# filaPro/unidet3d

Hardware: AMD Instinct MI355X
Metric: scenes/sec fwd+bwd, 100k-pt ScanNet voxel grid, 1/2/4/8 MI355X (higher is better)
Workload: dtype f32

## Files before the change

### unidet3d_amd/csrc/bn.hip

```cpp
#include <stdlib.h>

#include "u3d_common.h"

namespace u3d {

struct BnFin {
    double* sums;
    double rows;
    int set_rows;
    const float* gamma;
    const float* beta;
    float eps, momentum;
    float* running_mean;
    float* running_var;
    float* st;
    int64_t* nbt;
};

__device__ __forceinline__ void bn_finalize_channel(double s1, double s2, double rows, const float* gamma, const float* beta, float eps,
                                                    float momentum, float* running_mean, float* running_var, float* mean, float* invstd,
                                                    float* scale, float* shift, int c) {
#pragma clang fp contract(off)
    const double m = s1 / rows;
    double var = fma(-m, m, s2 / rows);
    if (var < 0.0) var = 0.0;
    const float is = (float)(1.0 / sqrt(var + (double)eps));
    const float mf = (float)m;
    mean[c] = mf;
    invstd[c] = is;
    const float sc = gamma[c] * is;
    scale[c] = sc;
    shift[c] = fmaf(-mf, sc, beta[c]);
    if (running_mean) {
        const double unbiased = rows > 1.0 ? var * rows / (rows - 1.0) : var;
        const float keep = 1.f - momentum;
        const float km = keep * running_mean[c], kv = keep * running_var[c];
        const float nm = momentum * mf, nv = momentum * (float)unbiased;
        running_mean[c] = km + nm;
        running_var[c] = kv + nv;
    }
}

__device__ __forceinline__ void bn_finish_body(const double* partial, int nblk, int C, const BnFin& f, int wave0, int nw, bool first) {
    const int lane = threadIdx.x & 63;
    for (int c = wave0; c < C; c += nw) {
        double t1 = 0.0, t2 = 0.0;
        for (int b = lane; b < nblk; b += 64) {
            t1 += partial[(int64_t)b * 2 * C + c];
            t2 += partial[(int64_t)b * 2 * C + C + c];
        }
#pragma unroll
        for (int d = 32; d >= 1; d >>= 1) { t1 += __shfl_xor(t1, d, 64); t2 += __shfl_xor(t2, d, 64); }
        if (lane) continue;
        f.sums[c] = t1;
        f.sums[C + c] = t2;
        if (!f.st) continue;
        bn_finalize_channel(t1, t2, f.rows, f.gamma, f.beta, f.eps, f.momentum, f.running_mean, f.running_var, f.st, f.st + C,
                            f.st + 2 * C, f.st + 3 * C, c);
    }
    if (first && threadIdx.x == 0) {
        if (f.set_rows) f.sums[2 * C] = f.rows;
        if (f.nbt) *f.nbt += 1;
    }
}

__global__ __launch_bounds__(256) void bn_sum_k(const double* __restrict__ partial, int nblk, int C, BnFin f) {
    bn_finish_body(partial, nblk, C, f, blockIdx.x * 4 + (threadIdx.x >> 6), gridDim.x * 4, blockIdx.x == 0);
}

template <int MODE>
__global__ __launch_bounds__(256) void bn_reduce_k(const float* __restrict__ x, const float* __restrict__ dy,
                                                   const float* __restrict__ mean, const float* __restrict__ invstd,
                                                   const float* __restrict__ scale, const float* __restrict__ shift, int relu,
                                                   int64_t n, int C, double* sums ) {
    __shared__ double sh[256 * 8];
    const int lpr = C >> 2;
    const int rpb = 256 / lpr;
    const int tid = threadIdx.x;
    const int c4 = tid % lpr, slot = tid / lpr;
    double a[4] = {0, 0, 0, 0}, b[4] = {0, 0, 0, 0};
    if (slot < rpb) {
        float4 mu = make_float4(0, 0, 0, 0), is = mu, sc = mu, sf = mu;
        if (MODE == 1) {
            mu = *reinterpret_cast<const float4*>(mean + c4 * 4);
            is = *reinterpret_cast<const float4*>(invstd + c4 * 4);
            sc = *reinterpret_cast<const float4*>(scale + c4 * 4);
            sf = *reinterpret_cast<const float4*>(shift + c4 * 4);
        }
        const int64_t stride = (int64_t)gridDim.x * rpb;
        for (int64_t r0 = (int64_t)blockIdx.x * rpb + slot; r0 < n; r0 += 4 * stride) {
            float4 v4[4], g4[4];
#pragma unroll
            for (int u = 0; u < 4; ++u) {
                const int64_t r = r0 + u * stride;
                v4[u] = make_float4(0.f, 0.f, 0.f, 0.f);
                g4[u] = make_float4(0.f, 0.f, 0.f, 0.f);
                if (r < n) {
                    v4[u] = *reinterpret_cast<const float4*>(x + r * C + c4 * 4);
                    if (MODE == 1) g4[u] = *reinterpret_cast<const float4*>(dy + r * C + c4 * 4);
                }
            }
#pragma unroll
            for (int u = 0; u < 4; ++u) {
                const float4 v = v4[u];
                if (MODE == 0) {
                    a[0] += v.x; a[1] += v.y; a[2] += v.z; a[3] += v.w;
                    b[0] += (double)v.x * v.x; b[1] += (double)v.y * v.y; b[2] += (double)v.z * v.z; b[3] += (double)v.w * v.w;
                } else {
                    float4 g = g4[u];
                    if (relu) {
                        if (!(v.x * sc.x + sf.x > 0.f)) g.x = 0.f;
                        if (!(v.y * sc.y + sf.y > 0.f)) g.y = 0.f;
                        if (!(v.z * sc.z + sf.z > 0.f)) g.z = 0.f;
                        if (!(v.w * sc.w + sf.w > 0.f)) g.w = 0.f;
                    }
                    a[0] += g.x; a[1] += g.y; a[2] += g.z; a[3] += g.w;
                    b[0] += (double)g.x * ((v.x - mu.x) * is.x); b[1] += (double)g.y * ((v.y - mu.y) * is.y);
                    b[2] += (double)g.z * ((v.z - mu.z) * is.z); b[3] += (double)g.w * ((v.w - mu.w) * is.w);
                }
            }
        }
    }
#pragma unroll
    for (int j = 0; j < 4; ++j) { sh[tid * 8 + j] = a[j]; sh[tid * 8 + 4 + j] = b[j]; }
    __syncthreads();
    if (tid < lpr) {
        double ta[4] = {0, 0, 0, 0}, tb[4] = {0, 0, 0, 0};
        for (int s = 0; s < rpb; ++s) {
            const int o = (s * lpr + tid) * 8;
#pragma unroll
            for (int j = 0; j < 4; ++j) { ta[j] += sh[o + j]; tb[j] += sh[o + 4 + j]; }
        }
        double* out = sums + (int64_t)blockIdx.x * 2 * C;
// ... 39 lines not shown
                              float* running_var, int C, float* mean, float* invstd, float* scale, float* shift,
                              int64_t* num_batches_tracked) {
    const int c = blockIdx.x * blockDim.x + threadIdx.x;
    if (c == 0 && num_batches_tracked) *num_batches_tracked += 1;
    if (c >= C) return;
    if (!(count > 0.0)) count = sums[2 * C];
    bn_finalize_channel(sums[c], sums[C + c], count, gamma, beta, eps, momentum, running_mean, running_var, mean, invstd, scale, shift, c);
}


__global__ __launch_bounds__(256) void bn_apply_k(const float* __restrict__ x, const float* __restrict__ scale,
                                                  const float* __restrict__ shift, int relu, int64_t n4, int C4, float* y, __bf16* yb) {
    for (int64_t i = (int64_t)blockIdx.x * blockDim.x + threadIdx.x; i < n4; i += (int64_t)gridDim.x * blockDim.x) {
        const int c4 = (int)(i % C4);
        const float4 v = reinterpret_cast<const float4*>(x)[i];
        const float4 sc = reinterpret_cast<const float4*>(scale)[c4];
        const float4 sf = reinterpret_cast<const float4*>(shift)[c4];
        const float4 o = bn_affine_relu(v, sc, sf, relu);
        reinterpret_cast<float4*>(y)[i] = o;
        if (yb) store_shadow(yb, i / C4, C4, 0, c4, o);
    }
}

__global__ __launch_bounds__(256) void bn_bwd_apply_k(const float* __restrict__ x, const float* __restrict__ dy,
                                                      const float* __restrict__ mean, const float* __restrict__ invstd,
                                                      const float* __restrict__ scale, const float* __restrict__ shift, int relu,
                                                      const double* __restrict__ sums, double inv_count, int64_t n4, int C,
                                                      float* dx, float* dgamma, float* dbeta, const double* __restrict__ count_src,
                                                      const float* __restrict__ addend, __bf16* dxb) {
    const int C4 = C >> 2;
    if (!(inv_count > 0.0)) inv_count = 1.0 / (count_src ? count_src[0] : sums[2 * C]);
    if (blockIdx.x == 0 && dgamma) {
        for (int c = threadIdx.x; c < C; c += blockDim.x) {
            dbeta[c] = (float)sums[c];
            dgamma[c] = (float)sums[C + c];
        }
    }
    for (int64_t i = (int64_t)blockIdx.x * blockDim.x + threadIdx.x; i < n4; i += (int64_t)gridDim.x * blockDim.x) {
        const int c4 = (int)(i % C4);
        const float4 v = reinterpret_cast<const float4*>(x)[i];
        float4 g = reinterpret_cast<const float4*>(dy)[i];
        const float4 mu = reinterpret_cast<const float4*>(mean)[c4];
        const float4 is = reinterpret_cast<const float4*>(invstd)[c4];
        const float4 sc = reinterpret_cast<const float4*>(scale)[c4];
        const float4 sf = reinterpret_cast<const float4*>(shift)[c4];
        if (relu) {
            if (!(v.x * sc.x + sf.x > 0.f)) g.x = 0.f;
            if (!(v.y * sc.y + sf.y > 0.f)) g.y = 0.f;
            if (!(v.z * sc.z + sf.z > 0.f)) g.z = 0.f;
            if (!(v.w * sc.w + sf.w > 0.f)) g.w = 0.f;
        }
        const int c = c4 * 4;
        const float m1x = (float)(sums[c] * inv_count), m1y = (float)(sums[c + 1] * inv_count);
        const float m1z = (float)(sums[c + 2] * inv_count), m1w = (float)(sums[c + 3] * inv_count);
        const float m2x = (float)(sums[C + c] * inv_count), m2y = (float)(sums[C + c + 1] * inv_count);
        const float m2z = (float)(sums[C + c + 2] * inv_count), m2w = (float)(sums[C + c + 3] * inv_count);
        float4 o;
        o.x = sc.x * (g.x - m1x - (v.x - mu.x) * is.x * m2x);
        o.y = sc.y * (g.y - m1y - (v.y - mu.y) * is.y * m2y);
        o.z = sc.z * (g.z - m1z - (v.z - mu.z) * is.z * m2z);
        o.w = sc.w * (g.w - m1w - (v.w - mu.w) * is.w * m2w);
        if (addend) {
            const float4 e = reinterpret_cast<const float4*>(addend)[i];
            o.x += e.x; o.y += e.y; o.z += e.z; o.w += e.w;
        }
        reinterpret_cast<float4*>(dx)[i] = o;
        if (dxb) store_shadow(dxb, i / C4, C4, 0, c4, o);
    }
}

static bool bn_ok(int64_t n, int C) { return n > 0 && C >= 4 && C <= 512 && C % 4 == 0; }
static bool shadow_ok(const void* sh, int C) { return !sh || C % 32 == 0; }
static unsigned ew_grid(int64_t n4) {
    int64_t g = ceil_div(n4, 256);
    return (unsigned)(g < 1 ? 1 : (g > 4096 ? 4096 : g));
}

}

using namespace u3d;

extern "C" {

static int bn_grid(int64_t n, int C) {
    const int rpb = 256 / (C / 4);
    int64_t g = ceil_div(n, (int64_t)rpb * 16);
    return (int)(g < 1 ? 1 : (g > 256 ? 256 : g));
}
static int bn_partials_grid(int64_t n_tiles, int C) {
    const int rpp = 2 * C >= 256 ? 1 : 256 / (2 * C);
    int64_t g = ceil_div(n_tiles, (int64_t)rpp * 16);
    return (int)(g < 1 ? 1 : (g > 128 ? 128 : g));
}

int64_t u3d_bn_ws_bytes(int C) { return (int64_t)256 * 2 * C * sizeof(double) + 64; }

static int bn_finish_launch(const void* ws, int nblk, int C, const BnFin& f, hipStream_t s) {
    hipLaunchKernelGGL(bn_sum_k, dim3((C + 3) / 4), dim3(256), 0, s, (const double*)ws, nblk, C, f);
    return check_launch("bn_sum");
}

static BnFin bn_fin(double* sums, double rows, int set_rows) {
    BnFin f;
    f.sums = sums; f.rows = rows; f.set_rows = set_rows; f.gamma = nullptr; f.beta = nullptr; f.eps = 0.f; f.momentum = 0.f;
    f.running_mean = nullptr; f.running_var = nullptr; f.st = nullptr; f.nbt = nullptr;
    return f;
}

static int bn_stats_launch(const float* x, int64_t n, int C, const float* partial, int64_t n_tiles, const BnFin& f, void* ws, hipStream_t s) {
    if (partial) {
        if (n_tiles <= 0) return U3D_EINVAL;
        ProfScope prof(U3D_K_BN, s, (double)n_tiles * C * 8);
        const int g = bn_partials_grid(n_tiles, C);
        hipLaunchKernelGGL(bn_partials_k, dim3(g), dim3(256), 0, s, partial, n_tiles, C, (double*)ws);
        return bn_finish_launch(ws, g, C, f, s);
    }
    ProfScope prof(U3D_K_BN, s, (double)n * C * 4);
    const int g = bn_grid(n, C);
    hipLaunchKernelGGL(bn_reduce_k<0>, dim3(g), dim3(256), 0, s, x, (const float*)nullptr, (const float*)nullptr,
                       (const float*)nullptr, (const float*)nullptr, (const float*)nullptr, 0, n, C, (double*)ws);
    return bn_finish_launch(ws, g, C, f, s);
}

int u3d_bn_stats(const float* x, int64_t n, int C, const float* partial, int64_t n_tiles, double* sums, void* ws, u3d_stream_t stream) {
    if ((!x && !partial) || !sums || !ws || !bn_ok(n, C)) return U3D_EINVAL;
    return bn_stats_launch(x, n, C, partial, n_tiles, bn_fin(sums, (double)n, 1), ws, (hipStream_t)stream);
}

int u3d_bn_finalize(const double* sums, double count, const float* gamma, const float* beta, float eps, float momentum,
                    float* running_mean, float* running_var, int C, float* mean, float* invstd, float* scale,
                    float* shift, int64_t* num_batches_tracked, u3d_stream_t stream) {
    if (!sums || !gamma || !beta || !mean || !invstd || !scale || !shift || C <= 0) return U3D_EINVAL;
    hipLaunchKernelGGL(bn_finalize_k, dim3((C + 63) / 64), dim3(64), 0, (hipStream_t)stream, sums, count, gamma, beta, eps,
                       momentum, running_mean, running_var, C, mean, invstd, scale, shift, num_batches_tracked);
    return check_launch("bn_finalize");
}

int u3d_bn_apply(const float* x, const float* scale, const float* shift, int relu, int64_t n, int C, float* y, void* y_bf16,
                 u3d_stream_t stream) {
    if (!x || !scale || !shift || !y || !bn_ok(n, C) || !shadow_ok(y_bf16, C)) return U3D_EINVAL;
    hipStream_t s = (hipStream_t)stream;
    ProfScope prof(U3D_K_BN, s, (double)n * C * (y_bf16 ? 10 : 8));
    const int64_t n4 = n * (C / 4);
    hipLaunchKernelGGL(bn_apply_k, dim3(ew_grid(n4)), dim3(256), 0, s, x, scale, shift, relu, n4, C / 4, y, (__bf16*)y_bf16);
    return check_launch("bn_apply");
}

int u3d_bn_bwd_stats(const float* x, const float* dy, const float* mean, const float* invstd, const float* scale,
                     const float* shift, int relu, int64_t n, int C, double* sums, void* ws, u3d_stream_t stream) {
    if (!x || !dy || !mean || !invstd || !scale || !shift || !sums || !ws || !bn_ok(n, C)) return U3D_EINVAL;
    hipStream_t s = (hipStream_t)stream;
    ProfScope prof(U3D_K_BN, s, (double)n * C * 8);
    const int g = bn_grid(n, C);
    const BnFin f = bn_fin(sums, 0.0, 0);
    hipLaunchKernelGGL(bn_reduce_k<1>, dim3(g), dim3(256), 0, s, x, dy, mean, invstd, scale, shift, relu, n, C, (double*)ws);
    return bn_finish_launch(ws, g, C, f, s);
}

int u3d_bn_bwd_apply(const float* x, const float* dy, const float* mean, const float* invstd, const float* scale,
                     const float* shift, int relu, const double* sums, double count, int64_t n, int C, float* dx, void* dx_bf16,
                     float* dgamma, float* dbeta, const float* addend, u3d_stream_t stream) {
    if (!x || !dy || !mean || !invstd || !scale || !shift || !sums || !dx || !bn_ok(n, C) || !shadow_ok(dx_bf16, C)) return U3D_EINVAL;
    hipStream_t s = (hipStream_t)stream;
    ProfScope prof(U3D_K_BN, s, (double)n * C * 12);
    const int64_t n4 = n * (C / 4);
    hipLaunchKernelGGL(bn_bwd_apply_k, dim3(ew_grid(n4)), dim3(256), 0, s, x, dy, mean, invstd, scale, shift, relu, sums,
                       1.0 / count, n4, C, dx, dgamma, dbeta, (const double*)nullptr, addend, (__bf16*)dx_bf16);
    return check_launch("bn_bwd_apply");
}

int u3d_bn_forward(const float* x, int64_t n, int C, const float* partial, int64_t n_tiles, const float* gamma, const float* beta, float eps,
                   float momentum, float* running_mean, float* running_var, int64_t* num_batches_tracked, int relu, float* y, void* y_bf16,
                   float* st, double* sums, void* ws, u3d_stream_t stream) {
    if (!x || !sums || !ws || !gamma || !beta || !st || !y || !bn_ok(n, C) || !shadow_ok(y_bf16, C)) return U3D_EINVAL;
    if (partial && n_tiles <= 0) return U3D_EINVAL;
    BnFin f = bn_fin(sums, (double)n, 1);
    f.gamma = gamma; f.beta = beta; f.eps = eps; f.momentum = momentum; f.running_mean = running_mean; f.running_var = running_var;
    f.st = st; f.nbt = num_batches_tracked;
    int rc = bn_stats_launch(x, n, C, partial, n_tiles, f, ws, (hipStream_t)stream);
    if (rc) return rc;
    return u3d_bn_apply(x, st + 2 * C, st + 3 * C, relu, n, C, y, y_bf16, stream);
}

int u3d_bn_backward(const float* x, const float* dy, const float* st, int relu, const double* fwd_sums, double* sums, int64_t n, int C,
                    float* dx, void* dx_bf16, float* dgamma, float* dbeta, const float* addend, void* ws, u3d_stream_t stream) {
    if (!fwd_sums || !st || !dx || !shadow_ok(dx_bf16, C)) return U3D_EINVAL;
    int rc = u3d_bn_bwd_stats(x, dy, st, st + C, st + 2 * C, st + 3 * C, relu, n, C, sums, ws, stream);
    if (rc) return rc;
    hipStream_t s = (hipStream_t)stream;
    ProfScope prof(U3D_K_BN, s, (double)n * C * 12);
    const int64_t n4 = n * (C / 4);
    hipLaunchKernelGGL(bn_bwd_apply_k, dim3(ew_grid(n4)), dim3(256), 0, s, x, dy, (const float*)st, (const float*)(st + C), (const float*)(st + 2 * C),
                       (const float*)(st + 3 * C), relu, (const double*)sums, -1.0, n4, C, dx, dgamma, dbeta, fwd_sums + 2 * C, addend,
                       (__bf16*)dx_bf16);
    return check_launch("bn_backward");
}

}
```

### unidet3d_amd/csrc/gemm.hip

```cpp
#include "gemm_common.h"

namespace u3d {

#define U3D_MFMA32(a, b, c) __builtin_amdgcn_mfma_f32_32x32x2f32((a), (b), (c), 0, 0, 0)

constexpr int GLD = GK + 4;


template <int TN, int EPI, int TM = GT>
__global__ __launch_bounds__(256) void gemm_nt_k(const float* __restrict__ A, const float* __restrict__ W, const float* __restrict__ bias,
                                                 float* __restrict__ C, int64_t M, int N, int K, const float* __restrict__ aux,
                                                 float* __restrict__ pre) {
    constexpr int NB = TN / 64, TA = TM / 64;
    __shared__ __attribute__((aligned(16))) float As[2][TM * GLD];
    __shared__ __attribute__((aligned(16))) float Bs[2][TN * GLD];
    const int tid = threadIdx.x, lane = tid & 63;
    const int wave = __builtin_amdgcn_readfirstlane(tid >> 6);
    const int wr = wave >> 1, wc = wave & 1, i32 = lane & 31, kh = lane >> 5;
    const int nt_ = (N + TN - 1) / TN;
    const int64_t wid_ = xcd_swizzle(blockIdx.x, gridDim.x);
    const int64_t m0 = (wid_ / nt_) * TM;
    const int n0 = (int)(wid_ % nt_) * TN;
    const int rows_a = (int)min((int64_t)TM, M - m0), rows_b = min(TN, N - n0);
    const __amdgpu_buffer_rsrc_t rs_a = make_rsrc(A + m0 * K, (int64_t)rows_a * K * 4);
// ... 473 lines not shown
    auto gload = [&](int t) {
#pragma unroll
        for (int j = 0; j < 4; ++j) {
            ra[j] = bload128(rs_a, ca ? va + j * 8 * N * 4 : va, t * (TKH * N * 4));
            rb[j] = bload128(rs_b, cb ? vb + j * 8 * K * 4 : vb, t * (TKH * K * 4));
        }
    };
    auto lstore = [&](int buf) {
#pragma unroll
        for (int j = 0; j < 4; ++j) {
            cs += ra[j];
            *reinterpret_cast<bf16x4*>(&As[buf][(srow + 8 * j) * TLH + sc4 * 4]) = bf16x4{(__bf16)ra[j][0], (__bf16)ra[j][1], (__bf16)ra[j][2], (__bf16)ra[j][3]};
            *reinterpret_cast<bf16x4*>(&Bs[buf][(srow + 8 * j) * TLH + sc4 * 4]) = bf16x4{(__bf16)rb[j][0], (__bf16)rb[j][1], (__bf16)rb[j][2], (__bf16)rb[j][3]};
        }
    };
    const int troff = ((lane & 15) >> 2) * TLH + 16 * ((lane >> 4) & 1) + 4 * (lane & 3);
    auto colfrag = [&](const __bf16* t, int row0, int col32) {
        const __bf16* p = t + row0 * TLH + col32 + troff;
        return tr16_pair(p, p + 4 * TLH);
    };
    f32x16 acc[2][2];
#pragma unroll
    for (int a = 0; a < 2; ++a)
#pragma unroll
        for (int b = 0; b < 2; ++b)
#pragma unroll
            for (int r = 0; r < 16; ++r) acc[a][b][r] = 0.f;
    const int nt = (rows + TKH - 1) / TKH;
    if (nt > 0) {
        gload(0);
        lstore(0);
    }
    __syncthreads();
    for (int t = 0; t < nt; ++t) {
        const int buf = t & 1;
        if (t + 1 < nt) gload(t + 1);
#pragma unroll
        for (int h = 0; h < 2; ++h) {
            const int r0 = h * 16 + kh * 8;
            bf16x8 af[2], bf[2];
#pragma unroll
            for (int u = 0; u < 2; ++u) {
                af[u] = colfrag(As[buf], r0, wr * 64 + u * 32);
                bf[u] = colfrag(Bs[buf], r0, wc * 64 + u * 32);
            }
#pragma unroll
            for (int a = 0; a < 2; ++a)
#pragma unroll
                for (int b = 0; b < 2; ++b) acc[a][b] = __builtin_amdgcn_mfma_f32_32x32x16_bf16(af[a], bf[b], acc[a][b], 0, 0, 0);
        }
        if (t + 1 < nt) lstore(buf ^ 1);
        __syncthreads();
    }
    const int64_t pstride = (int64_t)N * K + (colsum ? N : 0);
    const __amdgpu_buffer_rsrc_t rs_o = make_rsrc(partial + (int64_t)blockIdx.z * pstride, (int64_t)N * K * 4);
#pragma unroll
    for (int b = 0; b < 2; ++b) {
        const int k = k0 + wc * 64 + b * 32 + i32;
        const int vo = k < K ? ((n0 + 4 * kh) * K + k) * 4 : 0x7fffffff;
#pragma unroll
        for (int a = 0; a < 2; ++a)
#pragma unroll
            for (int r = 0; r < 16; ++r) {
                const int row = wr * 64 + a * 32 + (r & 3) + 8 * (r >> 2);
                float v = acc[a][b][r];
                asm volatile("" : "+v"(v));
                __builtin_amdgcn_raw_buffer_store_b32(__builtin_bit_cast(unsigned, v), rs_o, vo, row * K * 4, 0);
            }
    }
    if (colsum && blockIdx.y == 0) {
#pragma unroll
        for (int c = 0; c < 4; ++c) csum_s[srow][sc4 * 4 + c] = cs[c];
        __syncthreads();
        if (tid < GT && n0 + tid < N) {
            float v = 0.f;
#pragma unroll
            for (int r = 0; r < 8; ++r) v += csum_s[r][tid];
            partial[(int64_t)blockIdx.z * pstride + (int64_t)N * K + n0 + tid] = v;
        }
    }
}

__global__ __launch_bounds__(256) void gemm_tn_reduce_k(const float* __restrict__ partial, int S, int64_t n4, int64_t n4_main, float* __restrict__ C,
                                                        float* __restrict__ C2) {
    for (int64_t i = (int64_t)blockIdx.x * blockDim.x + threadIdx.x; i < n4; i += (int64_t)gridDim.x * blockDim.x) {
        float4 v[4];
#pragma unroll
        for (int u = 0; u < 4; ++u) v[u] = make_float4(0.f, 0.f, 0.f, 0.f);
        int s = 0;
        for (; s + 4 <= S; s += 4) {
#pragma unroll
            for (int u = 0; u < 4; ++u) {
                const float4 t = reinterpret_cast<const float4*>(partial)[(int64_t)(s + u) * n4 + i];
                v[u].x += t.x; v[u].y += t.y; v[u].z += t.z; v[u].w += t.w;
            }
        }
        for (; s < S; ++s) {
            const float4 t = reinterpret_cast<const float4*>(partial)[(int64_t)s * n4 + i];
            v[0].x += t.x; v[0].y += t.y; v[0].z += t.z; v[0].w += t.w;
        }
        float4* dst = i < n4_main ? reinterpret_cast<float4*>(C) + i : reinterpret_cast<float4*>(C2) + (i - n4_main);
        *dst = make_float4((v[0].x + v[1].x) + (v[2].x + v[3].x), (v[0].y + v[1].y) + (v[2].y + v[3].y),
                                                      (v[0].z + v[1].z) + (v[2].z + v[3].z), (v[0].w + v[1].w) + (v[2].w + v[3].w));
    }
}

void launch_tn_reduce(const float* ws, int S, int N, int K, float* C, float* colsum, hipStream_t s) {
    const int64_t n4_main = (int64_t)N * K / 4, n4 = n4_main + (colsum ? N / 4 : 0);
    int64_t grid = ceil_div(n4, 256);
    grid = grid > 1024 ? 1024 : grid;
    hipLaunchKernelGGL(gemm_tn_reduce_k, dim3((unsigned)grid), dim3(256), 0, s, ws, S, n4, n4_main, C, colsum);
}

__global__ __launch_bounds__(256) void gelu_fwd_k(const float4* __restrict__ h, float4* __restrict__ a, int64_t n4) {
    for (int64_t i = (int64_t)blockIdx.x * blockDim.x + threadIdx.x; i < n4; i += (int64_t)gridDim.x * blockDim.x) {
        const float4 v = h[i];
        a[i] = make_float4(gelu_f(v.x), gelu_f(v.y), gelu_f(v.z), gelu_f(v.w));
    }
}
__global__ __launch_bounds__(256) void gelu_bwd_k(const float4* __restrict__ da, const float4* __restrict__ h, float4* __restrict__ dh, int64_t n4) {
    for (int64_t i = (int64_t)blockIdx.x * blockDim.x + threadIdx.x; i < n4; i += (int64_t)gridDim.x * blockDim.x) {
        const float4 g = da[i], v = h[i];
        dh[i] = make_float4(g.x * gelu_grad_f(v.x), g.y * gelu_grad_f(v.y), g.z * gelu_grad_f(v.z), g.w * gelu_grad_f(v.w));
    }
}

__global__ __launch_bounds__(256) void transpose_k(const float* __restrict__ in, float* __restrict__ out, int R, int Ccols) {
    __shared__ float tile[32][33];
    const int bx = blockIdx.x * 32, by = blockIdx.y * 32;
    const int tx = threadIdx.x & 31, ty = threadIdx.x >> 5;
    for (int j = ty; j < 32; j += 8)
        if (by + j < R && bx + tx < Ccols) tile[j][tx] = in[(int64_t)(by + j) * Ccols + bx + tx];
    __syncthreads();
    for (int j = ty; j < 32; j += 8)
        if (bx + j < Ccols && by + tx < R) out[(int64_t)(bx + j) * R + by + tx] = tile[tx][j];
}

struct TrDesc { const float* src; float* dst; int64_t R, C, block0; };
__global__ __launch_bounds__(256) void transpose_batch_k(const TrDesc* __restrict__ desc, int n_desc) {
    __shared__ float tile[32][33];
    int lo = 0, hi = n_desc;
    while (hi - lo > 1) {
        const int mid = (lo + hi) >> 1;
        if (desc[mid].block0 <= (int64_t)blockIdx.x) lo = mid; else hi = mid;
    }
    const TrDesc d = desc[lo];
    const int R = (int)d.R, Ccols = (int)d.C;
    const int tiles_x = (Ccols + 31) / 32;
    const int rem = (int)((int64_t)blockIdx.x - d.block0);
    const int bx = (rem % tiles_x) * 32, by = (rem / tiles_x) * 32;
    const int tx = threadIdx.x & 31, ty = threadIdx.x >> 5;
    for (int j = ty; j < 32; j += 8)
        if (by + j < R && bx + tx < Ccols) tile[j][tx] = d.src[(int64_t)(by + j) * Ccols + bx + tx];
    __syncthreads();
    for (int j = ty; j < 32; j += 8)
        if (bx + j < Ccols && by + tx < R) d.dst[(int64_t)(bx + j) * R + by + tx] = tile[tx][j];
}

struct PlDesc { const float* src; bf16x8* dst; int64_t n8, block0; };
__global__ __launch_bounds__(256) void planes_batch_k(const PlDesc* __restrict__ desc, int n_desc) {
    int lo = 0, hi = n_desc;
    while (hi - lo > 1) {
        const int mid = (lo + hi) >> 1;
        if (desc[mid].block0 <= (int64_t)blockIdx.x) lo = mid; else hi = mid;
    }
    const PlDesc d = desc[lo];
    const int64_t idx = ((int64_t)blockIdx.x - d.block0) * 256 + threadIdx.x;
    if (idx >= d.n8) return;
    const f32x4 a = *reinterpret_cast<const f32x4*>(d.src + idx * 8), b = *reinterpret_cast<const f32x4*>(d.src + idx * 8 + 4);
    bf16x8 out[3];
    split3_x8(a, b, out);
#pragma unroll
    for (int q = 0; q < 3; ++q) d.dst[q * d.n8 + idx] = out[q];
}

static int tn_tile(int N, int K) { return ceil_div(N, GT) * ceil_div(K, GT) < 16 ? 64 : GT; }
static int tn_splits(int64_t M, int N, int K, int T, bool bf) {
    const int64_t tiles = ceil_div(N, T) * ceil_div(K, T);
    static const int target = [] { const char* e = getenv("U3D_TN_WGS"); return e && atoi(e) > 0 ? atoi(e) : 768; }();
    return tn_clamp_splits(ceil_div(bf ? 384 : target, tiles), M, GK);
}

static int nt_plan(int64_t M, int N, int K, bool bf, NtPlan* plan) {
    if (M <= 0 || N <= 0 || K <= 0) return U3D_EINVAL;
    const bool x3 = !bf && fp32_x3() && K % GKH == 0;
    if (K % (bf ? GKH : GK)) { set_error("gemm_nt: K=%d must be a multiple of %d", K, bf ? GKH : GK); return U3D_EUNSUPPORTED; }
    if (!nt_offsets_ok("gemm_nt", N, K)) return U3D_EUNSUPPORTED;
    static const int force = [] { const char* e = getenv("U3D_NT_TILE"); return e ? atoi(e) : 0; }();
    const double over[3] = {1.0, 1.04, 1.08};
    int best = 0;
    double best_t = 0.0;
    for (int c = x3 ? 1 : 0; c < 3; ++c) {
        const int64_t wgs = ceil_div(M, NT_TM[c]) * ceil_div(N, NT_TN[c]);
        const double t = (double)ceil_div(wgs, 256) * NT_TM[c] * NT_TN[c] * over[c];
// ... 220 lines not shown
```

### unidet3d_amd/csrc/spconv.hip

```cpp
#include <stdlib.h>

#include "u3d_common.h"
#include "spconv_gmm.h"

namespace u3d {

#ifndef U3D_GMM_ABL
#define U3D_GMM_ABL 0
#endif
#ifndef U3D_WG_ABL
#define U3D_WG_ABL 0
#endif
__device__ __forceinline__ int gmm_acc_idx(int r, int c4) { return GMM_SWZ ? r * 32 + ((c4 ^ (r & 7)) << 2) : r * GMM_ALD + (c4 << 2); }

template <int NI, int JB, int NW = 2>
struct GmmBuf {
    f32x4 a[NI];
    f32x4 b[JB][NW];
};

struct GmmItem {
    int k, base, e;
    bool valid;
};
// ... 626 lines not shown
                    for (int b = 0; b < NXW; ++b) asm volatile("" :: "v"(xv[u][b]));
                }
                return;
            }
#pragma unroll
            for (int u = 0; u < 4; ++u)
#pragma unroll
                for (int a = 0; a < NGW; ++a)
#pragma unroll
                    for (int b = 0; b < NXW; ++b) acc[a][b] = __builtin_amdgcn_mfma_f32_16x16x4f32(gv[u][a], xv[u][b], acc[a][b], 0, 0, 0);
        };
        load_idx(ioA, ixA, base);
        load_idx(ioB, ixB, min(base + 16, last));
        load_rows(gA, xA, ioA, ixA);
        for (int t = 0; t < nfull; t += 2) {
            load_rows(gB, xB, ioB, ixB);
            load_idx(ioA, ixA, min(base + (t + 2) * 16, last));
            mfmas(gA, xA);
            if (t + 1 >= nfull) break;
            load_rows(gA, xA, ioA, ixA);
            load_idx(ioB, ixB, min(base + (t + 3) * 16, last));
            mfmas(gB, xB);
        }
        base += nfull * 16;
    }
    if (base < hi) {
        float gv[4][NGW], xv[4][NXW];
#pragma unroll
        for (int u = 0; u < 4; ++u) {
            const int pi = min(base + 4 * q + u, hi - 1);
            const int io = bload32(rs_rg, pi * 4, ksoff), ix = bload32(rs_rx, pi * 4, ksoff);
            load_row_part<NGW>(gv[u], rs_g, (int)__umul24(io, CD * 4) + gvo);
            load_row_part<NXW>(xv[u], rs_x, (int)__umul24(ix, CS * 4) + xvo);
        }
#pragma unroll
        for (int u = 0; u < 4; ++u) {
            const bool ok = base + 4 * q + u < hi;
#pragma unroll
            for (int a = 0; a < NGW; ++a) {
                const float ga = ok ? gv[u][a] : 0.f;
#pragma unroll
                for (int b = 0; b < NXW; ++b) acc[a][b] = __builtin_amdgcn_mfma_f32_16x16x4f32(ga, xv[u][b], acc[a][b], 0, 0, 0);
            }
        }
    }
    if constexpr (LDSR) {
        constexpr int EW = NGW * NXW * 256;
        __shared__ float red[2][EW];
        float* mine = red[wave & 1] + lane;
        if (wave < 2) {
#pragma unroll
            for (int a = 0; a < NGW; ++a)
#pragma unroll
                for (int b = 0; b < NXW; ++b)
#pragma unroll
                    for (int r = 0; r < 4; ++r) mine[((a * NXW + b) * 4 + r) * 64] = acc[a][b][r];
        }
        __syncthreads();
        if (wave >= 2) {
#pragma unroll
            for (int a = 0; a < NGW; ++a)
#pragma unroll
                for (int b = 0; b < NXW; ++b)
#pragma unroll
                    for (int r = 0; r < 4; ++r) mine[((a * NXW + b) * 4 + r) * 64] += acc[a][b][r];
        }
        __syncthreads();
        const int group = range >> 2;
        if ((range & ~3) >= p.n_tiles) return;
        float* out = p.partial + ((int64_t)k * ceil_div(p.n_tiles, 4) + group) * (CD * CS);
        for (int e = threadIdx.x; e < EW; e += 256) out[e] = red[0][e] + red[1][e];
        return;
    }
    float* out = p.partial + ((int64_t)k * p.n_tiles + range) * (CD * CS) + (int64_t)sub * (NGW * NXW * 256) + lane;
#pragma unroll
    for (int a = 0; a < NGW; ++a)
#pragma unroll
        for (int b = 0; b < NXW; ++b)
#pragma unroll
            for (int r = 0; r < 4; ++r) out[((a * NXW + b) * 4 + r) * 64] = acc[a][b][r];
}

__global__ __launch_bounds__(256) void wgrad_reduce_k(const float* __restrict__ partial, int n_tiles, int K, int NG, int NX, int SG, int SX,
                                                      float* __restrict__ dW) {
    const int CS = NX * 16, E = NG * NX * 256;
    const int k = blockIdx.y;
    const int idx = blockIdx.x * 256 + threadIdx.x;
    if (idx >= E) return;
    const float* src = partial + (int64_t)k * n_tiles * E + idx;
    float v0 = 0.f, v1 = 0.f, v2 = 0.f, v3 = 0.f;
    int r = 0;
    for (; r + 4 <= n_tiles; r += 4) {
        v0 += src[(int64_t)r * E];
        v1 += src[(int64_t)(r + 1) * E];
        v2 += src[(int64_t)(r + 2) * E];
        v3 += src[(int64_t)(r + 3) * E];
    }
    for (; r < n_tiles; ++r) v0 += src[(int64_t)r * E];
    const float v = (v0 + v1) + (v2 + v3);
    const int NGW = NG / SG, NXW = NX / SX, per_sub = NGW * NXW * 256;
    const int sub = idx / per_sub, rem = idx % per_sub;
    const int e = rem >> 6, lane = rem & 63, i16 = lane & 15, q = lane >> 4;
    const int rr = e & 3, b = (e >> 2) % NXW, a = (e >> 2) / NXW;
    const int wa = sub % SG, wb = sub / SG;
    const int co = NG * (4 * q + rr) + wa * NGW + a, ci = NX * i16 + wb * NXW + b;
    dW[((int64_t)co * K + k) * CS + ci] = v;
}

static int plan_wgrad_rows(int K, int64_t n_rows, int Cs, int Cd) {
    static const int64_t cap = [] { const char* e = getenv("U3D_WGRAD_TILES"); const int64_t v = e ? atoll(e) : 0; return v > 0 ? v : (int64_t)256; }();
    static const int64_t budget = [] { const char* e = getenv("U3D_WGRAD_PARTIAL_MB"); const int64_t v = e ? atoll(e) : 0; return (v > 0 ? v : (int64_t)64) << 20; }();
    int64_t nt = budget / ((int64_t)K * Cs * Cd * 4);
    const int64_t rows_per = (K >= 27 && Cs == 32 && Cd == 32) ? 520 : 1300;
    const int64_t cap_n = cap > n_rows / rows_per ? cap : n_rows / rows_per;
    nt = nt > cap_n ? cap_n : (nt < 1 ? 1 : nt);
    const int64_t by_len = ceil_div(n_rows, 64);
    if (nt > by_len) nt = by_len;
    return (int)ceil_div(n_rows, nt);
}

template <int NX, int NG, int PR = 0>
static int launch_wgrad(const WgParams& p0, float* dW, hipStream_t s) {
    constexpr int SG = (NG * NX > 32 && NG % 2 == 0 && NG >= NX) ? 2 : ((NG * NX > 64 && NG % 2 == 0) ? 2 : 1);
    constexpr int SX = ((NG / SG) * NX > 32 && NX % 2 == 0) ? 2 : 1;
    constexpr int SPLIT = SG * SX, RPW = 4 / SPLIT;
    static_assert(SPLIT == 1 || SPLIT == 2 || SPLIT == 4, "wave split");
    const WgParams& p = p0;
    const int64_t groups = ceil_div(ceil_div(p.n_tiles, RPW), 8) * 8;
    static const int pipe_env = [] { const char* e = getenv("U3D_WGRAD_PIPE"); return e ? atoi(e) : -1; }();
    const bool pipe = pipe_env >= 0 ? pipe_env != 0 : (NG / SG) * (NX / SX) <= 16;
    if (pipe) hipLaunchKernelGGL((spconv_wgrad_k<NG, NX, SG, SX, PR, true>), dim3((unsigned)(groups * p.K)), dim3(256), 0, s, p);
    else hipLaunchKernelGGL((spconv_wgrad_k<NG, NX, SG, SX, PR, false>), dim3((unsigned)(groups * p.K)), dim3(256), 0, s, p);
    const int n_blocks = SPLIT == 1 ? (int)ceil_div(p.n_tiles, 4) : p.n_tiles;
    hipLaunchKernelGGL(wgrad_reduce_k, dim3(NG * NX, p.K), dim3(256), 0, s, (const float*)p.partial, n_blocks, p.K, NG, NX, SG, SX, dW);
    return check_launch("spconv_wgrad");
}

static inline int64_t weight_pack_vectors(int format, int Cd, int K, int Cs) { return (int64_t)(Cd / 32) * K * (Cs / (format ? 32 : 16)) * 2 * 64; }

__device__ __forceinline__ void weight_f32_vector(const float* __restrict__ w, float* __restrict__ wp, int64_t idx, int Cd, int K, int Cs, int transposed) {
    const int lane = (int)(idx & 63);
    int64_t t = idx >> 6;
    const int nb = (int)(t & 1); t >>= 1;
    const int cs16 = Cs / 16;
    if (idx >= (int64_t)(Cd / 32) * K * cs16 * 2 * 64) return;
    const int j = (int)(t % cs16); t /= cs16;
    const int k = (int)(t % K);
    const int slice = (int)(t / K);
    const int n = slice * 32 + nb * 16 + (lane & 15), c = j * 16 + (lane >> 4) * 4;
    float4 v;
    if (!transposed) {
        v = *reinterpret_cast<const float4*>(w + ((int64_t)n * K + k) * Cs + c);
    } else {
        v.x = w[((int64_t)(c + 0) * K + k) * Cd + n];
        v.y = w[((int64_t)(c + 1) * K + k) * Cd + n];
        v.z = w[((int64_t)(c + 2) * K + k) * Cd + n];
        v.w = w[((int64_t)(c + 3) * K + k) * Cd + n];
    }
    reinterpret_cast<float4*>(wp)[idx] = v;
}

__device__ __forceinline__ void weight_bf16_vector(const float* __restrict__ w, bf16x8* __restrict__ wp, int64_t idx, int Cd, int K, int Cs, int transposed) {
    const int lane = (int)(idx & 63);
    int64_t t = idx >> 6;
    const int nb = (int)(t & 1); t >>= 1;
    const int cs32 = Cs / 32;
    if (idx >= (int64_t)(Cd / 32) * K * cs32 * 2 * 64) return;
    const int jj = (int)(t % cs32); t /= cs32;
    const int k = (int)(t % K);
    const int slice = (int)(t / K);
    const int n = slice * 32 + nb * 16 + (lane & 15), q = lane >> 4;
    bf16x8 v;
#pragma unroll
    for (int e = 0; e < 8; ++e) {
        const int c = (2 * jj + (e >> 2)) * 16 + q * 4 + (e & 3);
        v[e] = (__bf16)(transposed ? w[((int64_t)c * K + k) * Cd + n] : w[((int64_t)n * K + k) * Cs + c]);
    }
    wp[idx] = v;
}

__device__ __forceinline__ void weight_x3_vectors(const float* __restrict__ w, bf16x8* __restrict__ wp, int64_t idx, int Cd, int K, int Cs, int transposed) {
    if (idx >= (int64_t)(Cd / 32) * K * (Cs / 32) * 2 * 64) return;
    const int cs32 = Cs / 32;
    const int lane = (int)(idx & 63);
    int64_t t = idx >> 6;
    const int nb = (int)(t & 1); t >>= 1;
    const int jj = (int)(t % cs32); t /= cs32;
    const int k = (int)(t % K);
    const int slice = (int)(t / K);
    const int n = slice * 32 + nb * 16 + (lane & 15), q = lane >> 4;
    float v[8];
#pragma unroll
    for (int e = 0; e < 8; ++e) {
        const int c = (2 * jj + (e >> 2)) * 16 + q * 4 + (e & 3);
        v[e] = transposed ? w[((int64_t)c * K + k) * Cd + n] : w[((int64_t)n * K + k) * Cs + c];
    }
    bf16x8 pl[3];
    split3_x8(f32x4{v[0], v[1], v[2], v[3]}, f32x4{v[4], v[5], v[6], v[7]}, pl);
    const int64_t o = (idx >> 6) * 192 + lane;
#pragma unroll
    for (int pq = 0; pq < 3; ++pq) wp[o + pq * 64] = pl[pq];
}
__device__ __forceinline__ void weight_pack_vector(int64_t format, const float* w, void* wp, int64_t idx, int Cd, int K, int Cs, int transposed) {
    if (format == 2) weight_x3_vectors(w, reinterpret_cast<bf16x8*>(wp), idx, Cd, K, Cs, transposed);
    else if (format) weight_bf16_vector(w, reinterpret_cast<bf16x8*>(wp), idx, Cd, K, Cs, transposed);
    else weight_f32_vector(w, reinterpret_cast<float*>(wp), idx, Cd, K, Cs, transposed);
}

template <int FORMAT>
__global__ __launch_bounds__(256) void weight_pack_k(const float* __restrict__ w, void* __restrict__ wp, int Cd, int K, int Cs, int transposed) {
    weight_pack_vector(FORMAT, w, wp, (int64_t)blockIdx.x * blockDim.x + threadIdx.x, Cd, K, Cs, transposed);
}

struct PackDesc { const float* src; void* dst; int64_t Cd, K, Cs, transposed, bf, block0; };
__global__ __launch_bounds__(256) void weight_pack_batch_k(const PackDesc* __restrict__ desc, int n_desc) {
    int lo = 0, hi = n_desc;
    while (hi - lo > 1) {
// ... 269 lines not shown
```

### unidet3d_amd/csrc/u3d_common.h

```cpp
#pragma once
#include <hip/hip_runtime.h>
#include <stdint.h>
#include <stdio.h>

#include <atomic>

#include "u3d.h"

namespace u3d {

void set_error(const char* fmt, ...);

struct ProfScope {
    int cls;
    hipStream_t stream;
    bool on;
    hipEvent_t e0, e1;
    double work;
    ProfScope(int cls, hipStream_t s, double work);
    ~ProfScope();
};

inline int check_launch(const char* what) {
    hipError_t e = hipGetLastError();
    if (e != hipSuccess) {
        set_error("%s: %s", what, hipGetErrorString(e));
        return U3D_ELAUNCH;
    }
    return U3D_OK;
}

__host__ __device__ inline int64_t ceil_div(int64_t a, int64_t b) { return (a + b - 1) / b; }

struct DeviceOnce {
    std::atomic<bool> flag[64];
    bool needed(int dev) const { return (unsigned)dev >= 64u || !flag[dev].load(std::memory_order_acquire); }
    void done(int dev) { if ((unsigned)dev < 64u) flag[dev].store(true, std::memory_order_release); }
};

__device__ __forceinline__ int64_t xcd_swizzle(int64_t b, int64_t n) {
    const int64_t q = n >> 3, r = n & 7, x = b & 7, i = b >> 3;
    return (x < r ? x * (q + 1) : r * (q + 1) + (x - r) * q) + i;
}

__device__ __forceinline__ float4 bn_affine_relu(const float4& v, const float4& sc, const float4& sf, int relu) {
    float4 o = make_float4(v.x * sc.x + sf.x, v.y * sc.y + sf.y, v.z * sc.z + sf.z, v.w * sc.w + sf.w);
    if (relu) { o.x = fmaxf(o.x, 0.f); o.y = fmaxf(o.y, 0.f); o.z = fmaxf(o.z, 0.f); o.w = fmaxf(o.w, 0.f); }
    return o;
}

using f32x4 = __attribute__((ext_vector_type(4))) float;
using u32x4 = __attribute__((ext_vector_type(4))) unsigned int;

#if defined(__HIP_DEVICE_COMPILE__) || defined(__HIPCC__)
__device__ __forceinline__ f32x4 bload128(__amdgpu_buffer_rsrc_t r, int voff, int soff) {
    return __builtin_bit_cast(f32x4, __builtin_amdgcn_raw_buffer_load_b128(r, voff, soff, 0));
}
__device__ __forceinline__ uint2 bload64(__amdgpu_buffer_rsrc_t r, int voff, int soff) {
    return __builtin_bit_cast(uint2, __builtin_amdgcn_raw_buffer_load_b64(r, voff, soff, 0));
}
__device__ __forceinline__ int bload32(__amdgpu_buffer_rsrc_t r, int voff, int soff) {
    return (int)__builtin_amdgcn_raw_buffer_load_b32(r, voff, soff, 0);
}
__device__ __forceinline__ __amdgpu_buffer_rsrc_t make_rsrc(const void* p, int64_t bytes = 0x7fffffff) {
    return __builtin_amdgcn_make_buffer_rsrc(const_cast<void*>(p), 0, (int)(bytes < 0x7fffffff ? bytes : 0x7fffffff), 0x00020000);
}
#endif

extern int g_fp32_math;
extern int g_conv_kernel;
extern int g_attn_tile_waves;
bool fp32_x3();
#if defined(__HIP_DEVICE_COMPILE__) || defined(__HIPCC__)
using u16x8 = __attribute__((ext_vector_type(8))) unsigned short;
using bf16x8 = __attribute__((ext_vector_type(8))) __bf16;
using bf16x4 = __attribute__((ext_vector_type(4))) __bf16;
using bf16x2 = __attribute__((ext_vector_type(2))) __bf16;
using s16x4 = __attribute__((ext_vector_type(4))) short;
using s16x8 = __attribute__((ext_vector_type(8))) short;
using f32x16 = __attribute__((ext_vector_type(16))) float;

__device__ __forceinline__ unsigned pack_bf16(float lo, float hi) { return __builtin_bit_cast(unsigned, bf16x2{(__bf16)lo, (__bf16)hi}); }
__device__ __forceinline__ float bf16_bits_to_f32(unsigned short b) { return __builtin_bit_cast(float, (unsigned)b << 16); }

__device__ __forceinline__ void store_shadow(__bf16* dst, int64_t row, int ld4, int col4, int c4, const float4& o) {
    const int g32 = c4 >> 3, half = (c4 >> 2) & 1, q = c4 & 3;
    reinterpret_cast<bf16x4*>(dst)[row * ld4 + col4 + g32 * 8 + q * 2 + half] = bf16x4{(__bf16)o.x, (__bf16)o.y, (__bf16)o.z, (__bf16)o.w};
}

__device__ __forceinline__ bf16x8 tr16_pair(const __bf16* p0, const __bf16* p1) {
    const s16x4 r0 = __builtin_amdgcn_ds_read_tr16_b64_v4i16((__attribute__((address_space(3))) s16x4*)p0);
    const s16x4 r1 = __builtin_amdgcn_ds_read_tr16_b64_v4i16((__attribute__((address_space(3))) s16x4*)p1);
    return __builtin_bit_cast(bf16x8, s16x8{r0[0], r0[1], r0[2], r0[3], r1[0], r1[1], r1[2], r1[3]});
}

__device__ __forceinline__ void gelu_parts(float x, float& cdf, float& pdf) {
    const float ax = fabsf(x), e = __expf(-0.5f * x * x);
    const float t = __frcp_rn(1.f + 0.3275911f * 0.70710678118654752440f * ax);
    const float poly = t * (0.254829592f + t * (-0.284496736f + t * (1.421413741f + t * (-1.453152027f + t * 1.061405429f))));
    const float tail = 0.5f * poly * e;
    cdf = x >= 0.f ? 1.f - tail : tail;
    pdf = 0.39894228040143267794f * e;
}
__device__ __forceinline__ float gelu_f(float x) { float c, p; gelu_parts(x, c, p); return x * c; }
__device__ __forceinline__ float gelu_grad_f(float x) { float c, p; gelu_parts(x, c, p); return c + x * p; }

__device__ __forceinline__ void split3_pair(float a, float b, unsigned& h, unsigned& m, unsigned& l) {
    const unsigned ah = (__builtin_bit_cast(unsigned, a) + 0x8000u) & 0xffff0000u, bh = (__builtin_bit_cast(unsigned, b) + 0x8000u) & 0xffff0000u;
    const float a1 = a - __builtin_bit_cast(float, ah), b1 = b - __builtin_bit_cast(float, bh);
    const unsigned a1b = __builtin_bit_cast(unsigned, a1), b1b = __builtin_bit_cast(unsigned, b1);
    const float a2 = a1 - __builtin_bit_cast(float, a1b & 0xffff0000u), b2 = b1 - __builtin_bit_cast(float, b1b & 0xffff0000u);
    h = __builtin_amdgcn_perm(bh, ah, 0x07060302u);
    m = __builtin_amdgcn_perm(b1b, a1b, 0x07060302u);
    l = __builtin_amdgcn_perm(__builtin_bit_cast(unsigned, b2), __builtin_bit_cast(unsigned, a2), 0x07060302u);
}
__device__ __forceinline__ void split3_x8(const f32x4& lo, const f32x4& hi, bf16x8 (&out)[3]) {
#ifdef U3D_SPLIT_ABL
    out[0] = __builtin_bit_cast(bf16x8, lo); out[1] = __builtin_bit_cast(bf16x8, hi); out[2] = out[0];
    return;
#endif
    unsigned w[3][4];
    split3_pair(lo[0], lo[1], w[0][0], w[1][0], w[2][0]);
    split3_pair(lo[2], lo[3], w[0][1], w[1][1], w[2][1]);
    split3_pair(hi[0], hi[1], w[0][2], w[1][2], w[2][2]);
    split3_pair(hi[2], hi[3], w[0][3], w[1][3], w[2][3]);
    u32x4 p[3];
#pragma unroll
    for (int q = 0; q < 3; ++q) p[q] = u32x4{w[q][0], w[q][1], w[q][2], w[q][3]};
#pragma unroll
    for (int q = 0; q < 3; ++q) out[q] = __builtin_bit_cast(bf16x8, p[q]);
}
#endif

int exclusive_scan_popc64(const uint64_t* words, int64_t n, int32_t* out, void* ws, hipStream_t s);
int exclusive_scan_i32(const int32_t* in, int64_t n, int32_t* out, void* ws, hipStream_t s);
// ... 56 lines not shown
```

Measured before the change: 309.3.

## Parallelize split-partial reductions with tree splitting and widen BN forward grid

Adds a shared helper that splits the partial-sum dimension across groups of threads in a block, with 8-way unrolled f32x4 loads, then combines the groups through shared memory. Both the GEMM TN split-K reduce and the sparse-conv weight-gradient reduce now use it, so small outputs with many partials still launch enough threads. The wgrad reduce is also vectorized to four elements per thread. BN forward stats may now use up to 512 partial blocks, and the finish kernel unrolls its loads when there are more than 256 partials. The trade-off is a larger BN workspace, extra synchronization, and a different summation order in float reductions.

```diff
diff --git a/unidet3d_amd/csrc/bn.hip b/unidet3d_amd/csrc/bn.hip
--- a/unidet3d_amd/csrc/bn.hip
+++ b/unidet3d_amd/csrc/bn.hip
@@ -41,14 +41,31 @@
     }
 }
 
+__device__ __forceinline__ void bn_lane_rows_x8(const double* partial, int nblk, int C, int c, int lane, double& t1, double& t2) {
+    for (int b0 = lane; b0 < nblk; b0 += 64 * 8) {
+        double p1[8], p2[8];
+#pragma unroll
+        for (int u = 0; u < 8; ++u) {
+            const int b = min(b0 + 64 * u, nblk - 1);
+            p1[u] = partial[(int64_t)b * 2 * C + c];
+            p2[u] = partial[(int64_t)b * 2 * C + C + c];
+        }
+#pragma unroll
+        for (int u = 0; u < 8; ++u)
+            if (b0 + 64 * u < nblk) { t1 += p1[u]; t2 += p2[u]; }
+    }
+}
+
 __device__ __forceinline__ void bn_finish_body(const double* partial, int nblk, int C, const BnFin& f, int wave0, int nw, bool first) {
     const int lane = threadIdx.x & 63;
     for (int c = wave0; c < C; c += nw) {
         double t1 = 0.0, t2 = 0.0;
-        for (int b = lane; b < nblk; b += 64) {
-            t1 += partial[(int64_t)b * 2 * C + c];
-            t2 += partial[(int64_t)b * 2 * C + C + c];
-        }
+        if (nblk > 256) bn_lane_rows_x8(partial, nblk, C, c, lane, t1, t2);
+        else
+            for (int b = lane; b < nblk; b += 64) {
+                t1 += partial[(int64_t)b * 2 * C + c];
+                t2 += partial[(int64_t)b * 2 * C + C + c];
+            }
 #pragma unroll
         for (int d = 32; d >= 1; d >>= 1) { t1 += __shfl_xor(t1, d, 64); t2 += __shfl_xor(t2, d, 64); }
         if (lane) continue;
@@ -254,10 +271,12 @@
 
 extern "C" {
 
-static int bn_grid(int64_t n, int C) {
+static const int BN_MAX_PARTIALS = 512;
+static const int BN_CAP[2] = {BN_MAX_PARTIALS, 256};
+static int bn_grid(int64_t n, int C, int mode) {
     const int rpb = 256 / (C / 4);
     int64_t g = ceil_div(n, (int64_t)rpb * 16);
-    return (int)(g < 1 ? 1 : (g > 256 ? 256 : g));
+    return (int)(g < 1 ? 1 : (g > BN_CAP[mode] ? BN_CAP[mode] : g));
 }
 static int bn_partials_grid(int64_t n_tiles, int C) {
     const int rpp = 2 * C >= 256 ? 1 : 256 / (2 * C);
@@ -265,7 +284,7 @@
     return (int)(g < 1 ? 1 : (g > 128 ? 128 : g));
 }
 
-int64_t u3d_bn_ws_bytes(int C) { return (int64_t)256 * 2 * C * sizeof(double) + 64; }
+int64_t u3d_bn_ws_bytes(int C) { return (int64_t)BN_MAX_PARTIALS * 2 * C * sizeof(double) + 64; }
 
 static int bn_finish_launch(const void* ws, int nblk, int C, const BnFin& f, hipStream_t s) {
     hipLaunchKernelGGL(bn_sum_k, dim3((C + 3) / 4), dim3(256), 0, s, (const double*)ws, nblk, C, f);
@@ -288,7 +307,7 @@
         return bn_finish_launch(ws, g, C, f, s);
     }
     ProfScope prof(U3D_K_BN, s, (double)n * C * 4);
-    const int g = bn_grid(n, C);
+    const int g = bn_grid(n, C, 0);
     hipLaunchKernelGGL(bn_reduce_k<0>, dim3(g), dim3(256), 0, s, x, (const float*)nullptr, (const float*)nullptr,
                        (const float*)nullptr, (const float*)nullptr, (const float*)nullptr, 0, n, C, (double*)ws);
     return bn_finish_launch(ws, g, C, f, s);
@@ -323,7 +342,7 @@
     if (!x || !dy || !mean || !invstd || !scale || !shift || !sums || !ws || !bn_ok(n, C)) return U3D_EINVAL;
     hipStream_t s = (hipStream_t)stream;
     ProfScope prof(U3D_K_BN, s, (double)n * C * 8);
-    const int g = bn_grid(n, C);
+    const int g = bn_grid(n, C, 1);
     const BnFin f = bn_fin(sums, 0.0, 0);
     hipLaunchKernelGGL(bn_reduce_k<1>, dim3(g), dim3(256), 0, s, x, dy, mean, invstd, scale, shift, relu, n, C, (double*)ws);
     return bn_finish_launch(ws, g, C, f, s);
diff --git a/unidet3d_amd/csrc/gemm.hip b/unidet3d_amd/csrc/gemm.hip
--- a/unidet3d_amd/csrc/gemm.hip
+++ b/unidet3d_amd/csrc/gemm.hip
@@ -579,34 +579,25 @@
 }
 
 __global__ __launch_bounds__(256) void gemm_tn_reduce_k(const float* __restrict__ partial, int S, int64_t n4, int64_t n4_main, float* __restrict__ C,
-                                                        float* __restrict__ C2) {
-    for (int64_t i = (int64_t)blockIdx.x * blockDim.x + threadIdx.x; i < n4; i += (int64_t)gridDim.x * blockDim.x) {
-        float4 v[4];
-#pragma unroll
-        for (int u = 0; u < 4; ++u) v[u] = make_float4(0.f, 0.f, 0.f, 0.f);
-        int s = 0;
-        for (; s + 4 <= S; s += 4) {
-#pragma unroll
-            for (int u = 0; u < 4; ++u) {
-                const float4 t = reinterpret_cast<const float4*>(partial)[(int64_t)(s + u) * n4 + i];
-                v[u].x += t.x; v[u].y += t.y; v[u].z += t.z; v[u].w += t.w;
-            }
-        }
-        for (; s < S; ++s) {
-            const float4 t = reinterpret_cast<const float4*>(partial)[(int64_t)s * n4 + i];
-            v[0].x += t.x; v[0].y += t.y; v[0].z += t.z; v[0].w += t.w;
-        }
-        float4* dst = i < n4_main ? reinterpret_cast<float4*>(C) + i : reinterpret_cast<float4*>(C2) + (i - n4_main);
-        *dst = make_float4((v[0].x + v[1].x) + (v[2].x + v[3].x), (v[0].y + v[1].y) + (v[2].y + v[3].y),
-                                                      (v[0].z + v[1].z) + (v[2].z + v[3].z), (v[0].w + v[1].w) + (v[2].w + v[3].w));
+                                                        float* __restrict__ C2, int parts) {
+    __shared__ f32x4 sh[256];
+    const int W = 256 / parts;
+    for (int64_t base = (int64_t)blockIdx.x * W; base < n4; base += (int64_t)gridDim.x * W) {
+        const int64_t i = base + threadIdx.x % W;
+        const bool active = i < n4;
+        const f32x4 v = reduce_tree_f4(reinterpret_cast<const f32x4*>(partial) + (active ? i : 0), n4, S, parts, active, sh);
+        if (!active || threadIdx.x >= W) continue;
+        f32x4* dst = i < n4_main ? reinterpret_cast<f32x4*>(C) + i : reinterpret_cast<f32x4*>(C2) + (i - n4_main);
+        *dst = v;
     }
 }
 
 void launch_tn_reduce(const float* ws, int S, int N, int K, float* C, float* colsum, hipStream_t s) {
     const int64_t n4_main = (int64_t)N * K / 4, n4 = n4_main + (colsum ? N / 4 : 0);
-    int64_t grid = ceil_div(n4, 256);
-    grid = grid > 1024 ? 1024 : grid;
-    hipLaunchKernelGGL(gemm_tn_reduce_k, dim3((unsigned)grid), dim3(256), 0, s, ws, S, n4, n4_main, C, colsum);
+    const int parts = reduce_tree_parts(S);
+    int64_t grid = ceil_div(n4, 256 / parts);
+    grid = grid > 65536 ? 65536 : grid;
+    hipLaunchKernelGGL(gemm_tn_reduce_k, dim3((unsigned)grid), dim3(256), 0, s, ws, S, n4, n4_main, C, colsum, parts);
 }
 
 __global__ __launch_bounds__(256) void gelu_fwd_k(const float4* __restrict__ h, float4* __restrict__ a, int64_t n4) {
diff --git a/unidet3d_amd/csrc/spconv.hip b/unidet3d_amd/csrc/spconv.hip
--- a/unidet3d_amd/csrc/spconv.hip
+++ b/unidet3d_amd/csrc/spconv.hip
@@ -732,29 +732,28 @@
 }
 
 __global__ __launch_bounds__(256) void wgrad_reduce_k(const float* __restrict__ partial, int n_tiles, int K, int NG, int NX, int SG, int SX,
-                                                      float* __restrict__ dW) {
-    const int CS = NX * 16, E = NG * NX * 256;
+                                                      float* __restrict__ dW, int parts) {
+    __shared__ f32x4 sh[256];
+    const int CS = NX * 16, E4 = NG * NX * 64;
     const int k = blockIdx.y;
-    const int idx = blockIdx.x * 256 + threadIdx.x;
-    if (idx >= E) return;
-    const float* src = partial + (int64_t)k * n_tiles * E + idx;
-    float v0 = 0.f, v1 = 0.f, v2 = 0.f, v3 = 0.f;
-    int r = 0;
-    for (; r + 4 <= n_tiles; r += 4) {
-        v0 += src[(int64_t)r * E];
-        v1 += src[(int64_t)(r + 1) * E];
-        v2 += src[(int64_t)(r + 2) * E];
-        v3 += src[(int64_t)(r + 3) * E];
-    }
-    for (; r < n_tiles; ++r) v0 += src[(int64_t)r * E];
-    const float v = (v0 + v1) + (v2 + v3);
+    const int W = 256 / parts;
+    const int j = blockIdx.x * W + threadIdx.x % W;
+    const bool active = j < E4;
+    const f32x4* src = reinterpret_cast<const f32x4*>(partial) + (int64_t)k * n_tiles * E4 + (active ? j : 0);
+    const f32x4 v = reduce_tree_f4(src, E4, n_tiles, parts, active, sh);
+    if (!active || threadIdx.x >= W) return;
     const int NGW = NG / SG, NXW = NX / SX, per_sub = NGW * NXW * 256;
+    const int idx = j * 4;
     const int sub = idx / per_sub, rem = idx % per_sub;
-    const int e = rem >> 6, lane = rem & 63, i16 = lane & 15, q = lane >> 4;
+    const int e = rem >> 6, lane = rem & 63, q = lane >> 4;
     const int rr = e & 3, b = (e >> 2) % NXW, a = (e >> 2) / NXW;
     const int wa = sub % SG, wb = sub / SG;
-    const int co = NG * (4 * q + rr) + wa * NGW + a, ci = NX * i16 + wb * NXW + b;
-    dW[((int64_t)co * K + k) * CS + ci] = v;
+    const int co = NG * (4 * q + rr) + wa * NGW + a;
+#pragma unroll
+    for (int c = 0; c < 4; ++c) {
+        const int i16 = (lane & 15) + c, ci = NX * i16 + wb * NXW + b;
+        dW[((int64_t)co * K + k) * CS + ci] = v[c];
+    }
 }
 
 static int plan_wgrad_rows(int K, int64_t n_rows, int Cs, int Cd) {
@@ -782,7 +781,9 @@
     if (pipe) hipLaunchKernelGGL((spconv_wgrad_k<NG, NX, SG, SX, PR, true>), dim3((unsigned)(groups * p.K)), dim3(256), 0, s, p);
     else hipLaunchKernelGGL((spconv_wgrad_k<NG, NX, SG, SX, PR, false>), dim3((unsigned)(groups * p.K)), dim3(256), 0, s, p);
     const int n_blocks = SPLIT == 1 ? (int)ceil_div(p.n_tiles, 4) : p.n_tiles;
-    hipLaunchKernelGGL(wgrad_reduce_k, dim3(NG * NX, p.K), dim3(256), 0, s, (const float*)p.partial, n_blocks, p.K, NG, NX, SG, SX, dW);
+    const int parts = reduce_tree_parts(n_blocks);
+    hipLaunchKernelGGL(wgrad_reduce_k, dim3((unsigned)ceil_div(NG * NX * 64, 256 / parts), p.K), dim3(256), 0, s, (const float*)p.partial, n_blocks,
+                       p.K, NG, NX, SG, SX, dW, parts);
     return check_launch("spconv_wgrad");
 }
 
diff --git a/unidet3d_amd/csrc/u3d_common.h b/unidet3d_amd/csrc/u3d_common.h
--- a/unidet3d_amd/csrc/u3d_common.h
+++ b/unidet3d_amd/csrc/u3d_common.h
@@ -51,6 +51,43 @@
 
 using f32x4 = __attribute__((ext_vector_type(4))) float;
 using u32x4 = __attribute__((ext_vector_type(4))) unsigned int;
+
+__device__ __forceinline__ f32x4 reduce_run_f4(const f32x4* __restrict__ src, int64_t stride, int lo, int hi) {
+    f32x4 v[8];
+#pragma unroll
+    for (int u = 0; u < 8; ++u) v[u] = f32x4{0.f, 0.f, 0.f, 0.f};
+    int s = lo;
+    for (; s + 8 <= hi; s += 8) {
+        f32x4 t[8];
+#pragma unroll
+        for (int u = 0; u < 8; ++u) t[u] = src[(int64_t)(s + u) * stride];
+#pragma unroll
+        for (int u = 0; u < 8; ++u) v[u] += t[u];
+    }
+    if (s < hi) {
+        f32x4 t[8];
+#pragma unroll
+        for (int u = 0; u < 8; ++u) t[u] = src[(int64_t)min(s + u, hi - 1) * stride];
+#pragma unroll
+        for (int u = 0; u < 8; ++u) v[u] += s + u < hi ? t[u] : f32x4{0.f, 0.f, 0.f, 0.f};
+    }
+    return ((v[0] + v[1]) + (v[2] + v[3])) + ((v[4] + v[5]) + (v[6] + v[7]));
+}
+
+__device__ __forceinline__ f32x4 reduce_tree_f4(const f32x4* __restrict__ src, int64_t stride, int count, int parts, bool active, f32x4* sh) {
+    const int W = 256 / parts, e = threadIdx.x % W, p = threadIdx.x / W;
+    const int len = (count + parts - 1) / parts;
+    const int lo = active ? min(p * len, count) : 0, hi = active ? min(lo + len, count) : 0;
+    f32x4 v = reduce_run_f4(src, stride, lo, hi);
+    if (parts == 1) return v;
+    sh[threadIdx.x] = v;
+    __syncthreads();
+    if (p == 0)
+        for (int q = 1; q < parts; ++q) v += sh[q * W + e];
+    __syncthreads();
+    return v;
+}
+static inline int reduce_tree_parts(int count) { return count >= 64 ? 16 : (count >= 8 ? 4 : 1); }
 
 #if defined(__HIP_DEVICE_COMPILE__) || defined(__HIPCC__)
 __device__ __forceinline__ f32x4 bload128(__amdgpu_buffer_rsrc_t r, int voff, int soff) {
```

Measured after the change: 309.2. No clear change (-0.0%).
